# bigscience-workshop/petals

Hardware: AMD Instinct MI355X
Metric: single-batch generate tokens/sec, Llama-2-70B across 1/2/4/8 MI355X servers (higher is better)
Workload: dtype nf4-weights/bf16-compute; 1 GPU; model=llama-2-70b, global_batch=1, seq_len=363, prompt_len=128, parallelism=swarm-single, quant=nf4, stack=serve

## Files before the change

petals_amd/ops/csrc/bindings.cpp:

```cpp
#include <torch/extension.h>
#include <ATen/cuda/CUDAContext.h>

torch::Tensor rms_norm(torch::Tensor x, torch::Tensor w, double eps);
torch::Tensor rms_norm_f32out(torch::Tensor x, torch::Tensor w, double eps);
torch::Tensor layer_norm(torch::Tensor x, torch::Tensor w, torch::Tensor b, double eps);
torch::Tensor layer_norm_f32out(torch::Tensor x, torch::Tensor w, torch::Tensor b, double eps);
torch::Tensor swiglu(torch::Tensor gate, torch::Tensor up);
void warm_spin(int64_t microseconds);
std::vector<torch::Tensor> apply_rope(
    torch::Tensor q, torch::Tensor k, torch::Tensor cos_t, torch::Tensor sin_t, torch::Tensor pos);
void rope_cache_write(
    torch::Tensor qkv, torch::Tensor cos_t, torch::Tensor sin_t, torch::Tensor pos,
    torch::Tensor k_cache, torch::Tensor v_cache, int64_t qh, int64_t kh);
void kv_cache_write(
    torch::Tensor qkv, torch::Tensor pos,
    torch::Tensor k_cache, torch::Tensor v_cache, int64_t qh, int64_t kh);
void kv_cache_store_fp8(torch::Tensor new_kv, torch::Tensor cache, int64_t prefix_length);
torch::Tensor qkv_rope_reduce(
    torch::Tensor partials, c10::optional<torch::Tensor> cos_t, c10::optional<torch::Tensor> sin_t,
    torch::Tensor pos, torch::Tensor k_cache, torch::Tensor v_cache,
    int64_t qh, int64_t kh, bool rope, c10::optional<torch::Tensor> bias);
torch::Tensor gemv_bf16(
    torch::Tensor wt, torch::Tensor x, torch::Tensor workspace,
    c10::optional<torch::Tensor> residual, int64_t epilogue, int64_t splits_override,
    c10::optional<torch::Tensor> bias);
torch::Tensor attn_decode_fused(
    torch::Tensor q, torch::Tensor k_cache, torch::Tensor v_cache, torch::Tensor kv_len,
    int64_t gq, int64_t n_splits, torch::Tensor part_o, torch::Tensor part_ml, double scale,
    c10::optional<torch::Tensor> alibi_slopes);
torch::Tensor attn_prefill_fused(
    torch::Tensor q, torch::Tensor k, torch::Tensor v,
    int64_t kv_len, int64_t kv_offset, double scale, bool causal,
    c10::optional<torch::Tensor> alibi_slopes);
std::vector<torch::Tensor> nf4_quantize(torch::Tensor w);
torch::Tensor gemv_int8(
    torch::Tensor q, torch::Tensor scale, torch::Tensor x, torch::Tensor workspace,
    c10::optional<torch::Tensor> residual, int64_t epilogue, int64_t splits_override,
    c10::optional<torch::Tensor> bias);
torch::Tensor nf4_dequantize(torch::Tensor packed, torch::Tensor absmax);
torch::Tensor gemv_nf4(
    torch::Tensor packed, torch::Tensor absmax, torch::Tensor x, torch::Tensor workspace,
    c10::optional<torch::Tensor> residual, int64_t epilogue, int64_t splits_override,
    c10::optional<torch::Tensor> bias, c10::optional<torch::Tensor> absmax_t);
torch::Tensor gemv_bf16_moe(
    torch::Tensor wt_all, torch::Tensor x, torch::Tensor sel, int64_t k_per_tok,
    torch::Tensor workspace, int64_t epilogue, int64_t splits_override);
torch::Tensor gemv_nf4_moe(
    torch::Tensor packed_all, torch::Tensor absmax_all, torch::Tensor x, torch::Tensor sel,
    int64_t k_per_tok, torch::Tensor workspace, int64_t epilogue, int64_t splits_override);
torch::Tensor moe_gemm(
    c10::optional<torch::Tensor> wt_all, c10::optional<torch::Tensor> packed_all,
    c10::optional<torch::Tensor> absmax_all, torch::Tensor x, torch::Tensor sorted_pairs,
    torch::Tensor tile_expert, int64_t k_per_tok, int64_t n_rows,
    c10::optional<torch::Tensor> q8_all, c10::optional<torch::Tensor> scale8_all);
torch::Tensor gemv_int8_moe(
    torch::Tensor q8_all, torch::Tensor scale8_all, torch::Tensor x, torch::Tensor sel,
    int64_t k_per_tok, torch::Tensor workspace, int64_t epilogue, int64_t splits_override);
int64_t gemv_int8_moe_splits(int64_t in_dim, int64_t out_dim, int64_t rows, int64_t splits_override);
torch::Tensor gemm_nf4(
    torch::Tensor packed, torch::Tensor absmax, torch::Tensor x, c10::optional<torch::Tensor> bias);
torch::Tensor gemm_int8(
    torch::Tensor q8, torch::Tensor scale8, torch::Tensor x, c10::optional<torch::Tensor> bias);
std::vector<torch::Tensor> mxfp4_quantize(torch::Tensor w);
torch::Tensor mxfp4_dequantize(torch::Tensor packed, torch::Tensor scales);
torch::Tensor gemv_mxfp4(
    torch::Tensor packed, torch::Tensor scales, torch::Tensor x, torch::Tensor workspace,
    c10::optional<torch::Tensor> residual, int64_t epilogue, int64_t splits_override,
    c10::optional<torch::Tensor> bias);
int64_t gemv_mxfp4_splits(int64_t in_dim, int64_t out_dim, int64_t batch, int64_t splits_override);
torch::Tensor gemm_mxfp4(
    torch::Tensor packed, torch::Tensor scales, torch::Tensor x, c10::optional<torch::Tensor> bias);

PYBIND11_MODULE(TORCH_EXTENSION_NAME, m) {
  m.def("rms_norm", &rms_norm, "RMSNorm (bf16 -> bf16)");
  m.def("rms_norm_f32out", &rms_norm_f32out, "RMSNorm (bf16 -> f32)");
  m.def("layer_norm", &layer_norm, "LayerNorm with weight+bias (bf16 -> bf16)");
  m.def("layer_norm_f32out", &layer_norm_f32out, "LayerNorm with weight+bias (bf16 -> f32)");
  m.def("swiglu", &swiglu, "silu(gate) * up (bf16)");
  m.def("warm_spin", &warm_spin, "occupy the device queue for ~N us (keep-warm)");
  m.def("apply_rope", &apply_rope, "rotate q,k by positions (bf16)");
  m.def("rope_cache_write", &rope_cache_write, "fused decode rope + kv cache write");
  m.def("kv_cache_write", &kv_cache_write, "decode kv cache write without rope (ALiBi families)");
  m.def("kv_cache_store_fp8", &kv_cache_store_fp8,
        "prefill write bf16 [B, KV, S, hd] -> float8_e4m3fn cache rows [prefix, prefix+S) "
        "(saturating, round to nearest even)",
        py::arg("new_kv"), py::arg("cache"), py::arg("prefix_length"));
  m.def("qkv_rope_reduce", &qkv_rope_reduce,
        "fused qkv split-K reduce + rope + kv-cache write (consumes RAW gemv partials)",
        py::arg("partials"), py::arg("cos_t"), py::arg("sin_t"), py::arg("pos"),
        py::arg("k_cache"), py::arg("v_cache"), py::arg("qh"), py::arg("kh"), py::arg("rope") = true,
        py::arg("bias") = py::none());
  m.def("gemv_bf16", &gemv_bf16, "split-K bf16 gemv with fused epilogue",
        py::arg("wt"), py::arg("x"), py::arg("workspace"), py::arg("residual"), py::arg("epilogue"),
        py::arg("splits") = 0, py::arg("bias") = py::none());
  m.def("attn_decode_fused", &attn_decode_fused, "GQA decode attention (flash-decoding)",
        py::arg("q"), py::arg("k_cache"), py::arg("v_cache"), py::arg("kv_len"), py::arg("gq"),
        py::arg("n_splits"), py::arg("part_o"), py::arg("part_ml"), py::arg("scale"),
        py::arg("alibi_slopes") = py::none());
  m.def("attn_prefill_fused", &attn_prefill_fused, "MFMA flash prefill attention (bf16, causal, GQA)",
        py::arg("q"), py::arg("k"), py::arg("v"), py::arg("kv_len"), py::arg("kv_offset"),
        py::arg("scale"), py::arg("causal"), py::arg("alibi_slopes") = py::none());
  m.def("gemv_int8", &gemv_int8, "split-K weight-only int8 gemv (per-column scales) with epilogue",
        py::arg("q"), py::arg("scale"), py::arg("x"), py::arg("workspace"),
        py::arg("residual"), py::arg("epilogue"), py::arg("splits") = 0, py::arg("bias") = py::none());
  m.def("nf4_quantize", &nf4_quantize, "blockwise NF4 quantize [in,out] bf16 -> (packed u8, absmax bf16)");
  m.def("nf4_dequantize", &nf4_dequantize, "NF4 -> bf16");
  m.def("gemv_nf4", &gemv_nf4, "split-K NF4 gemv (dequant fused) with epilogue",
        py::arg("packed"), py::arg("absmax"), py::arg("x"), py::arg("workspace"),
        py::arg("residual"), py::arg("epilogue"), py::arg("splits") = 0, py::arg("bias") = py::none(),
        py::arg("absmax_t") = py::none());
  m.def("gemv_bf16_moe", &gemv_bf16_moe,
        "device-routed MoE gemv: stacked bf16 expert weights, expert ids from a device tensor",
        py::arg("wt_all"), py::arg("x"), py::arg("sel"), py::arg("k_per_tok"),
        py::arg("workspace"), py::arg("epilogue"), py::arg("splits") = 0);
  m.def("gemv_nf4_moe", &gemv_nf4_moe,
        "device-routed MoE gemv: stacked NF4 expert weights, expert ids from a device tensor",
        py::arg("packed_all"), py::arg("absmax_all"), py::arg("x"), py::arg("sel"),
        py::arg("k_per_tok"), py::arg("workspace"), py::arg("epilogue"), py::arg("splits") = 0);
  m.def("moe_gemm", &moe_gemm,
        "grouped MFMA GEMM over expert-sorted (token, slot) pairs (prefill; NF4/int8 dequant "
        "fused into the LDS B-tile staging); exactly one of wt_all / packed_all / q8_all",
        py::arg("wt_all"), py::arg("packed_all"), py::arg("absmax_all"), py::arg("x"),
        py::arg("sorted_pairs"), py::arg("tile_expert"), py::arg("k_per_tok"), py::arg("n_rows"),
        py::arg("q8_all") = py::none(), py::arg("scale8_all") = py::none());
  m.def("gemv_int8_moe", &gemv_int8_moe,
        "device-routed MoE gemv: stacked int8 expert weights (per-column scales), expert ids "
        "from a device tensor",
        py::arg("q8_all"), py::arg("scale8_all"), py::arg("x"), py::arg("sel"),
        py::arg("k_per_tok"), py::arg("workspace"), py::arg("epilogue"), py::arg("splits") = 0);
  m.def("gemv_int8_moe_splits", &gemv_int8_moe_splits,
        "split count gemv_int8_moe uses for (in, out, rows) — sizes the workspace",
        py::arg("in_dim"), py::arg("out_dim"), py::arg("rows"), py::arg("splits") = 0);
  m.def("gemm_nf4", &gemm_nf4,
        "dense prefill MFMA GEMM x[M,in] @ NF4 W[in,out] (+bias) -> bf16, dequant fused into the "
        "LDS staging",
        py::arg("packed"), py::arg("absmax"), py::arg("x"), py::arg("bias") = py::none());
  m.def("gemm_int8", &gemm_int8,
        "dense prefill MFMA GEMM x[M,in] @ int8 W[in,out] (+bias) -> bf16, column scale in the "
        "epilogue",
        py::arg("q8"), py::arg("scale8"), py::arg("x"), py::arg("bias") = py::none());
  m.def("mxfp4_quantize", &mxfp4_quantize,
        "OCP MXFP4 quantize [in,out] bf16 -> (packed u8 [in/2,out], E8M0 scales u8 [in/32,out])");
  m.def("mxfp4_dequantize", &mxfp4_dequantize, "MXFP4 -> bf16 [in,out]");
  m.def("gemv_mxfp4", &gemv_mxfp4,
        "split-K MXFP4 gemv (hardware fp4 dequant, E8M0 block scales) with epilogue",
        py::arg("packed"), py::arg("scales"), py::arg("x"), py::arg("workspace"),
        py::arg("residual"), py::arg("epilogue"), py::arg("splits") = 0, py::arg("bias") = py::none());
  m.def("gemv_mxfp4_splits", &gemv_mxfp4_splits,
        "split count gemv_mxfp4 uses for (in, out, batch) — sizes the workspace",
        py::arg("in_dim"), py::arg("out_dim"), py::arg("batch"), py::arg("splits") = 0);
  m.def("gemm_mxfp4", &gemm_mxfp4,
        "dense prefill MFMA GEMM x[M,in] @ MXFP4 W[in,out] (+bias) -> bf16, hardware fp4 dequant "
        "fused into the LDS staging",
        py::arg("packed"), py::arg("scales"), py::arg("x"), py::arg("bias") = py::none());
}
```

petals_amd/ops/csrc/nf4.hip:

```cpp

#include "common.h"
#include "gemv_reduce.h"
#include <torch/extension.h>
#include <ATen/cuda/CUDAContext.h>

__device__ __constant__ float NF4_LUT_C[16] = {
    -1.0f, -0.6961928009986877f, -0.5250730514526367f, -0.39491748809814453f,
    -0.28444138169288635f, -0.18477343022823334f, -0.09105003625154495f, 0.0f,
    0.07958029955625534f, 0.16093020141124725f, 0.24611230194568634f,
    0.33791524171829224f, 0.4407098293304443f, 0.5626170039176941f,
    0.7229568362236023f, 1.0f};


__global__ void nf4_quantize_kernel(
    const unsigned short* __restrict__ w,
    unsigned char* __restrict__ packed,
    unsigned short* __restrict__ absmax,
    long n_blocks,
    int out_dim) {
  const long blk = (long)blockIdx.x * blockDim.x + threadIdx.x;
  if (blk >= n_blocks) return;
  const long base = blk * 64;
  float vals[64];
  float amax = 0.f;
#pragma unroll
  for (int j = 0; j < 64; ++j) {
    vals[j] = bf16_to_f32(w[base + j]);
    amax = fmaxf(amax, fabsf(vals[j]));
  }
  const float amax_bf = bf16_to_f32(f32_to_bf16(amax));
  absmax[blk] = f32_to_bf16(amax);
  const float inv = amax_bf > 0.f ? 1.0f / amax_bf : 0.f;
#pragma unroll
  for (int j = 0; j < 32; ++j) {
    unsigned char lo, hi;
#pragma unroll
    for (int half = 0; half < 2; ++half) {
      const float v = vals[2 * j + half] * inv;
      int best = 0;
      float bd = fabsf(v - NF4_LUT_C[0]);
#pragma unroll
      for (int l = 1; l < 16; ++l) {
        const float d = fabsf(v - NF4_LUT_C[l]);
        if (d < bd) { bd = d; best = l; }
      }
      if (half == 0) lo = (unsigned char)best; else hi = (unsigned char)best;
    }
    packed[blk * 32 + j] = (unsigned char)(lo | (hi << 4));
  }
}


__global__ void nf4_dequant_kernel(
    const unsigned char* __restrict__ packed,
    const unsigned short* __restrict__ absmax,
    unsigned short* __restrict__ out,
    long n_elems) {
  const long i = ((long)blockIdx.x * blockDim.x + threadIdx.x) * 2;
  if (i >= n_elems) return;
  const unsigned char byte = packed[i >> 1];
  const float scale = bf16_to_f32(absmax[i >> 6]);
  out[i] = f32_to_bf16(NF4_LUT_C[byte & 0xF] * scale);
  if (i + 1 < n_elems) out[i + 1] = f32_to_bf16(NF4_LUT_C[byte >> 4] * scale);
}


#define NF4_OPL 8
#define NF4_OUT_PER_WAVE (WAVE * NF4_OPL)

template <int BATCH>
__global__ __launch_bounds__(WAVE) void gemv_nf4_kernel(
    const unsigned char* __restrict__ packed,
    const unsigned short* __restrict__ absmax,
    const unsigned short* __restrict__ absmax_t,
    const float* __restrict__ x,
    float* __restrict__ partials,
    int in_dim,
    int out_dim,
    int i_per_split) {
  __shared__ float2 lut2[256];
  for (int i = threadIdx.x; i < 256; i += blockDim.x)
    lut2[i] = make_float2(NF4_LUT_C[i & 0xF], NF4_LUT_C[i >> 4]);
  __syncthreads();

  constexpr int OPL = NF4_OPL;
  const int lane = threadIdx.x & (WAVE - 1);
  const int out0 = blockIdx.x * (WAVE * OPL) + lane * OPL;
  if (out0 >= out_dim) return;
  const int split = blockIdx.y;
  const int i_begin = split * i_per_split;
  const int i_end = min(i_begin + i_per_split, in_dim);
  const bool full = (out0 + OPL) <= out_dim;

  float acc[BATCH][OPL];
#pragma unroll
  for (int b = 0; b < BATCH; ++b)
#pragma unroll
    for (int v = 0; v < OPL; ++v) acc[b][v] = 0.f;

  if (full) {
    constexpr int UNROLL = (BATCH > 4) ? 8 : 16;
    const int half_out = out_dim >> 1;
    const unsigned char* pp = packed + (size_t)i_begin * half_out + (out0 >> 1);
    const unsigned short* amt = absmax_t ? absmax_t + (size_t)(out0 >> 6) * in_dim : nullptr;
    int i = i_begin;
    for (; i + UNROLL <= i_end; i += UNROLL) {
      unsigned int pk[UNROLL];
#pragma unroll
      for (int u = 0; u < UNROLL; ++u)
        pk[u] = *reinterpret_cast<const unsigned int*>(pp + (size_t)u * half_out);
      float am[UNROLL];
      if (amt) {
#pragma unroll
        for (int c8 = 0; c8 < UNROLL / 8; ++c8) {
          const short8 a8 = *reinterpret_cast<const short8*>(amt + i + c8 * 8);
#pragma unroll
          for (int e = 0; e < 8; ++e) am[c8 * 8 + e] = bf16_to_f32((unsigned short)a8[e]);
        }
      } else {
#pragma unroll
        for (int u = 0; u < UNROLL; ++u)
          am[u] = bf16_to_f32(absmax[(size_t)(i + u) * (out_dim >> 6) + (out0 >> 6)]);
      }
      float xs[BATCH][UNROLL];
#pragma unroll
      for (int b = 0; b < BATCH; ++b)
#pragma unroll
        for (int u = 0; u < UNROLL; ++u)
          xs[b][u] = x[(size_t)b * in_dim + i + u];
#pragma unroll
      for (int u = 0; u < UNROLL; ++u) {
        float wf[OPL];
#pragma unroll
        for (int p2 = 0; p2 < 4; ++p2) {
          const float2 w2 = lut2[(pk[u] >> (8 * p2)) & 0xFFu];
          wf[2 * p2] = w2.x;
          wf[2 * p2 + 1] = w2.y;
        }
#pragma unroll
        for (int b = 0; b < BATCH; ++b) {
          const float xa = xs[b][u] * am[u];
#pragma unroll
          for (int v = 0; v < OPL; ++v) acc[b][v] = fmaf(wf[v], xa, acc[b][v]);
        }
      }
      pp += (size_t)UNROLL * half_out;
    }
    for (; i < i_end; ++i) {
      const float am = bf16_to_f32(absmax[(size_t)i * (out_dim >> 6) + (out0 >> 6)]);
#pragma unroll
      for (int b = 0; b < BATCH; ++b) {
        const float xa = x[(size_t)b * in_dim + i] * am;
        const unsigned int wd =
            *reinterpret_cast<const unsigned int*>(packed + (size_t)i * half_out + (out0 >> 1));
#pragma unroll
        for (int p2 = 0; p2 < 4; ++p2) {
          const float2 w2 = lut2[(wd >> (8 * p2)) & 0xFFu];
          acc[b][2 * p2] = fmaf(w2.x, xa, acc[b][2 * p2]);
          acc[b][2 * p2 + 1] = fmaf(w2.y, xa, acc[b][2 * p2 + 1]);
        }
      }
    }
  } else {
    for (int i = i_begin; i < i_end; ++i) {
      const float am = bf16_to_f32(absmax[(size_t)i * (out_dim >> 6) + (out0 >> 6)]);
#pragma unroll
      for (int b = 0; b < BATCH; ++b) {
        const float xa = x[(size_t)b * in_dim + i] * am;
#pragma unroll
        for (int v = 0; v < OPL; ++v) {
          if (out0 + v < out_dim) {
            const unsigned char byte = packed[(size_t)i * (out_dim >> 1) + ((out0 + v) >> 1)];
            const float2 w2 = lut2[byte];
            acc[b][v] = fmaf(((out0 + v) & 1) ? w2.y : w2.x, xa, acc[b][v]);
          }
        }
      }
    }
  }

#pragma unroll
  for (int b = 0; b < BATCH; ++b) {
    float* dst = partials + ((size_t)split * BATCH + b) * out_dim + out0;
    if (full) {
#pragma unroll
      for (int q = 0; q < OPL / 4; ++q)
        reinterpret_cast<float4v*>(dst)[q] =
            float4v{acc[b][4 * q], acc[b][4 * q + 1], acc[b][4 * q + 2], acc[b][4 * q + 3]};
    } else {
#pragma unroll
      for (int v = 0; v < OPL; ++v)
        if (out0 + v < out_dim) dst[v] = acc[b][v];
    }
  }
}


std::vector<torch::Tensor> nf4_quantize(torch::Tensor w) {
  TORCH_CHECK(w.is_cuda() && w.dtype() == torch::kBFloat16 && w.dim() == 2);
  TORCH_CHECK(w.size(1) % 64 == 0, "out dim must be a multiple of 64");
  auto wc = w.contiguous();
  const long in_dim = wc.size(0), out_dim = wc.size(1);
  const long n_blocks = in_dim * out_dim / 64;
  auto packed = torch::empty({in_dim, out_dim / 2}, w.options().dtype(torch::kUInt8));
  auto absmax = torch::empty({in_dim, out_dim / 64}, w.options());
  auto stream = at::cuda::getCurrentCUDAStream();
  const long blocks = (n_blocks + 255) / 256;
  nf4_quantize_kernel<<<blocks, 256, 0, stream>>>(
      reinterpret_cast<const unsigned short*>(wc.data_ptr()),
      packed.data_ptr<unsigned char>(),
      reinterpret_cast<unsigned short*>(absmax.data_ptr()),
      n_blocks, (int)out_dim);
  HIP_CHECK_LAST();
  return {packed, absmax};
}

torch::Tensor nf4_dequantize(torch::Tensor packed, torch::Tensor absmax) {
  TORCH_CHECK(packed.is_cuda() && packed.dtype() == torch::kUInt8 && packed.dim() == 2);
  const long in_dim = packed.size(0), half_out = packed.size(1);
  const long n = in_dim * half_out * 2;
  auto out = torch::empty({in_dim, half_out * 2}, absmax.options());
  auto stream = at::cuda::getCurrentCUDAStream();
  const long blocks = (n / 2 + 255) / 256;
  nf4_dequant_kernel<<<blocks, 256, 0, stream>>>(
      packed.data_ptr<unsigned char>(),
      reinterpret_cast<const unsigned short*>(absmax.data_ptr()),
      reinterpret_cast<unsigned short*>(out.data_ptr()), n);
  HIP_CHECK_LAST();
  return out;
}

torch::Tensor gemv_nf4(
    torch::Tensor packed,
    torch::Tensor absmax,
    torch::Tensor x,
    torch::Tensor workspace,
    c10::optional<torch::Tensor> residual,
    int64_t epilogue,
    int64_t splits_override,
    c10::optional<torch::Tensor> bias,
    c10::optional<torch::Tensor> absmax_t) {
  TORCH_CHECK(packed.is_cuda() && packed.dtype() == torch::kUInt8);
  TORCH_CHECK(x.dtype() == torch::kFloat32 && x.dim() == 2);
  const int in_dim = packed.size(0);
  const int out_dim = packed.size(1) * 2;
  const int batch = x.size(0);
  TORCH_CHECK(x.size(1) == in_dim && batch <= 8, "NF4 decode gemv supports batch <= 8");

  const long out_waves = (out_dim + (long)NF4_OUT_PER_WAVE - 1) / NF4_OUT_PER_WAVE;
  long splits = splits_override > 0 ? splits_override : (1536 + out_waves - 1) / out_waves;
  long max_splits = (in_dim + 31) / 32;
  if (splits > max_splits) splits = max_splits;
  if (splits < 1) splits = 1;
  const int i_per_split = (int)(((in_dim + splits - 1) / splits + 15L) & ~15L);
  splits = (in_dim + i_per_split - 1) / i_per_split;

  torch::Tensor partials;
  auto f32opts = x.options().dtype(torch::kFloat32);
  if (workspace.numel() >= (int64_t)splits * batch * out_dim) {
    partials = workspace;
  } else {
    partials = torch::empty({(int64_t)splits, batch, out_dim}, f32opts);
  }
  dim3 grid(out_waves, splits);
  auto stream = at::cuda::getCurrentCUDAStream();

  const unsigned short* amt_p = nullptr;
  if (absmax_t.has_value() && absmax_t->defined() && absmax_t->numel() > 0) {
    TORCH_CHECK(absmax_t->is_contiguous() && absmax_t->size(0) == out_dim / 64
                && absmax_t->size(1) == in_dim);
    amt_p = reinterpret_cast<const unsigned short*>(absmax_t->data_ptr());
  }
#define LAUNCH_NF4(B)                                                         \
  case B:                                                                     \
    gemv_nf4_kernel<B><<<grid, WAVE, 0, stream>>>(                            \
        packed.data_ptr<unsigned char>(),                                     \
        reinterpret_cast<const unsigned short*>(absmax.data_ptr()), amt_p,    \
        x.data_ptr<float>(), partials.data_ptr<float>(), in_dim, out_dim, i_per_split); \
    break;
  switch (batch) {
    LAUNCH_NF4(1) LAUNCH_NF4(2) LAUNCH_NF4(3) LAUNCH_NF4(4)
    LAUNCH_NF4(5) LAUNCH_NF4(6) LAUNCH_NF4(7) LAUNCH_NF4(8)
  }
#undef LAUNCH_NF4
  HIP_CHECK_LAST();

  if (epilogue < 0) {
    return partials.view(-1).narrow(0, 0, (int64_t)splits * batch * out_dim)
        .view({(int64_t)splits, (int64_t)batch, (int64_t)out_dim});
  }
  return launch_gemv_reduce(
      partials, residual, bias, (int)splits, batch, out_dim, (int)epilogue, f32opts,
      absmax.options());
}
```

petals_amd/ops/fused_decode.py:

```python

from __future__ import annotations

import math
import os
from typing import Dict, Optional, Tuple

import torch

from petals_amd.ops import reference

_EPI_RAW = -1
_EPI_PLAIN_F32 = 0
_EPI_PLAIN_BF16 = 1
_EPI_RESIDUAL_BF16 = 2
_EPI_SWIGLU_F32 = 3
_EPI_GELU_F32 = 4

_workspaces: Dict[Tuple[torch.device, str], torch.Tensor] = {}
_retired_workspaces: list = []


def _get_ws(device: torch.device, key: str, numel: int) -> torch.Tensor:
    k = (device, key)
    ws = _workspaces.get(k)
    if ws is None or ws.numel() < numel:
        if ws is not None:
            _retired_workspaces.append(ws)
        ws = torch.empty(numel, dtype=torch.float32, device=device)
        _workspaces[k] = ws
    return ws


class DecodeContext:

    def __init__(self, device: torch.device):
        self.pos = torch.zeros(1, dtype=torch.int32, device=device)
        self.kv_len = torch.zeros(1, dtype=torch.int32, device=device)

    def set_position(self, prefix_length: int) -> None:
        self.pos.fill_(prefix_length)
        self.kv_len.fill_(prefix_length + 1)

    def advance(self) -> None:
        self.pos.add_(1)
        self.kv_len.add_(1)


_split_autotune_cache: Dict[Tuple[str, int, int], int] = {}

_PREFILL_GEMM_MODES = ("dense", "fused")


def prefill_gemm_mode() -> str:
    mode = os.environ.get("PETALS_AMD_PREFILL_GEMM", "dense")
    if mode not in _PREFILL_GEMM_MODES:
        raise ValueError(
            f"PETALS_AMD_PREFILL_GEMM={mode!r}: expected one of {', '.join(_PREFILL_GEMM_MODES)}"
        )
    return mode


def set_prefill_gemm_mode(mode: str) -> None:
    if mode not in _PREFILL_GEMM_MODES:
        raise ValueError(f"prefill_gemm={mode!r}: expected one of {', '.join(_PREFILL_GEMM_MODES)}")
    os.environ["PETALS_AMD_PREFILL_GEMM"] = mode


FUSED_GEMM_MAX_ROWS = {"nf4": 256, "int8": 512, "mxfp4": 256}


def fused_gemm_eligible(quant: str, rows: int, in_dim: int, out_dim: int) -> bool:
    return (
        quant in FUSED_GEMM_MAX_ROWS
        and 1 <= rows <= FUSED_GEMM_MAX_ROWS[quant]
        and in_dim % 64 == 0
        and out_dim % 64 == 0
    )


class _FastWeight:

    def __init__(self, t_bf16: torch.Tensor, hip, quant: str):
        self.hip = hip
        self.quant = quant
        self.in_dim, self.out_dim = t_bf16.shape
        self.t = self.packed = self.absmax = self.absmax_t = self.q8 = self.scale8 = None
        self.mx_packed = self.mx_scales = None
        if quant == "mxfp4":
            from petals_amd.ops import mxfp4

            mxfp4.check_shape(self.in_dim, self.out_dim)
            if t_bf16.is_cuda:
                self.mx_packed, self.mx_scales = hip.mxfp4_quantize(t_bf16.to(torch.bfloat16).contiguous())
            else:
                self.mx_packed, self.mx_scales = mxfp4.quantize(t_bf16.to(torch.bfloat16))
        elif quant == "nf4":
            self.packed, self.absmax = hip.nf4_quantize(t_bf16.contiguous())
            self.absmax_t = self.absmax.t().contiguous()
        elif quant == "int8":
            w = t_bf16.float()
            scale = w.abs().amax(dim=0).clamp_min(1e-8) / 127.0
            self.q8 = torch.round(w / scale).clamp(-127, 127).to(torch.int8).contiguous()
            self.scale8 = scale.to(torch.bfloat16).contiguous()
        else:
            self.t = t_bf16.contiguous()
        self.splits = self._autotune(t_bf16.device)

    def _autotune(self, device) -> int:
        key = (self.quant, self.in_dim, self.out_dim)
        if key in _split_autotune_cache:
            return _split_autotune_cache[key]
        if device.type != "cuda":
            return 0
        import time

        if self.quant == "nf4":
            candidates = [0, 32, 64, 96, 128, 160, 192, 256, 320, 384]
            max_chunk = 32
        elif self.quant == "int8":
            candidates = [0, 16, 32, 64, 128, 192]
            max_chunk = 128
        elif self.quant == "mxfp4":
            candidates = [0, 8, 16, 24, 32, 48, 64]
            max_chunk = 32
        else:
            candidates = [0, 8, 16, 32, 64, 128]
            max_chunk = 64
        candidates = [s for s in candidates if s == 0 or s * max_chunk <= self.in_dim]
        x = torch.randn(1, self.in_dim, device=device)
        ws = _get_ws(device, "gemv", 64 * max(self.out_dim, 1))
        best, best_t = 0, float("inf")
        for s in candidates:
            try:
                self._gemv_raw(x, ws, None, 0, s)
                torch.cuda.synchronize()
                t0 = time.perf_counter()
                for _ in range(8):
                    self._gemv_raw(x, ws, None, 0, s)
                torch.cuda.synchronize()
                dt = time.perf_counter() - t0
            except RuntimeError:
                continue
            if dt < best_t:
                best, best_t = s, dt
        _split_autotune_cache[key] = best
        return best

    @property
    def shape(self):
        return (self.in_dim, self.out_dim)

    def _gemv_raw(self, x, ws, residual, epilogue, splits, bias=None):
        if self.quant == "nf4":
            return self.hip.gemv_nf4(self.packed, self.absmax, x, ws, residual, epilogue, splits, bias,
                                     self.absmax_t)
        if self.quant == "int8":
            return self.hip.gemv_int8(self.q8, self.scale8, x, ws, residual, epilogue, splits, bias)
        if self.quant == "mxfp4":
            return self.hip.gemv_mxfp4(self.mx_packed, self.mx_scales, x, ws, residual, epilogue, splits, bias)
        return self.hip.gemv_bf16(self.t, x, ws, residual, epilogue, splits, bias)

    def gemv(self, x, ws, residual, epilogue, bias=None):
        return self._gemv_raw(x, ws, residual, epilogue, self.splits, bias)

    def dense(self) -> torch.Tensor:
        if self.quant == "nf4":
            return _dequant_cached(self, lambda: self.hip.nf4_dequantize(self.packed, self.absmax))
        if self.quant == "int8":
            return _dequant_cached(
                self, lambda: (self.q8.to(torch.float32) * self.scale8.float()).to(torch.bfloat16)
            )
        if self.quant == "mxfp4":
            if not self.mx_packed.is_cuda:
                from petals_amd.ops import mxfp4

                return mxfp4.dequantize(self.mx_packed, self.mx_scales)
            return _dequant_cached(self, lambda: self.hip.mxfp4_dequantize(self.mx_packed, self.mx_scales))
        return self.t

    def matmul(self, x: torch.Tensor, bias: Optional[torch.Tensor] = None) -> torch.Tensor:
        if (
            prefill_gemm_mode() == "fused"
            and not (torch.is_grad_enabled() and x.requires_grad)
            and x.is_cuda
            and x.dtype == torch.bfloat16
            and fused_gemm_eligible(self.quant, x.numel() // max(x.shape[-1], 1), self.in_dim, self.out_dim)
        ):
            x2 = x.reshape(-1, self.in_dim).contiguous()
            if self.quant == "nf4":
                out = self.hip.gemm_nf4(self.packed, self.absmax, x2, bias)
            elif self.quant == "mxfp4":
                out = self.hip.gemm_mxfp4(self.mx_packed, self.mx_scales, x2, bias)
            else:
                out = self.hip.gemm_int8(self.q8, self.scale8, x2, bias)
            return out.view(*x.shape[:-1], self.out_dim)
        out = torch.matmul(x, self.dense())
        return out if bias is None else out + bias


_dequant_cache: "OrderedDict[int, torch.Tensor]" = None
_dequant_cache_bytes = 0


def _dequant_cache_budget() -> int:
    import os as _os

    return int(_os.environ.get("PETALS_AMD_DEQUANT_CACHE_MB", "16384")) << 20


def _dequant_cached(w, make) -> torch.Tensor:
    global _dequant_cache, _dequant_cache_bytes
    from collections import OrderedDict

    if _dequant_cache is None:
        _dequant_cache = OrderedDict()
    key = id(w)
    t = _dequant_cache.get(key)
    if t is not None:
        _dequant_cache.move_to_end(key)
        return t
    t = make()
    budget = _dequant_cache_budget()
    nbytes = t.numel() * t.element_size()
    if nbytes > budget:
        return t
    while _dequant_cache and _dequant_cache_bytes + nbytes > budget:
        _k, old = _dequant_cache.popitem(last=False)
        _dequant_cache_bytes -= old.numel() * old.element_size()
    _dequant_cache[key] = t
    _dequant_cache_bytes += nbytes
    import weakref

    def _evict(k=key):
        global _dequant_cache_bytes
        old = _dequant_cache.pop(k, None) if _dequant_cache else None
        if old is not None:
            _dequant_cache_bytes -= old.numel() * old.element_size()

    weakref.finalize(w, _evict)
    return t


def decode_step_auto(fast, hidden, k_cache, v_cache, prefix_length: int = -1, ctx=None, adapter=None,
                     max_b: int = 8):
    B = hidden.shape[0]
    if B <= max_b:
        return fast.decode_step(hidden, k_cache, v_cache, prefix_length, ctx=ctx, adapter=adapter)
    outs = []
    for i in range(0, B, max_b):
        outs.append(
            fast.decode_step(
                hidden[i : i + max_b], k_cache[i : i + max_b], v_cache[i : i + max_b],
                prefix_length, ctx=ctx, adapter=adapter,
            )
        )
    return torch.cat(outs, dim=0)


class _TPFastPathMixin:

    tp_world = 1
    tp_group = None

    @staticmethod
    def _mm_autograd(w: "_FastWeight", x: torch.Tensor, bias: Optional[torch.Tensor] = None) -> torch.Tensor:
        out = torch.matmul(x, w.dense())
        return out if bias is None else out + bias

    def _tp_copy(self, x: torch.Tensor) -> torch.Tensor:
        if self.tp_world <= 1:
            return x
        from petals_amd.parallel.tp import copy_to_tp

        return copy_to_tp(x, self.tp_group)

    def _tp_allreduce_(self, t: torch.Tensor) -> None:
        import torch.distributed as dist

        dist.all_reduce(t, op=dist.ReduceOp.SUM, group=self.tp_group)

    def _tp_reduce(self, x: torch.Tensor) -> torch.Tensor:
        if self.tp_world <= 1:
            return x
        from petals_amd.parallel.tp import reduce_from_tp

        return reduce_from_tp(x, self.tp_group)


class LlamaFastPath(_TPFastPathMixin):
    graph_safe = True

    def __init__(self, block, hip_ops, quant: str = "none", tp_world: int = 1, tp_group=None):
        cfg = block.config
        self.hip = hip_ops
        self.cfg = cfg
        self.quant = quant
        self.tp_world = tp_world
        self.tp_group = tp_group
        if tp_world > 1:
            self.graph_safe = False
        self.hd = cfg.head_dim
        self.qh = cfg.num_attention_heads
        self.kh = cfg.n_kv_heads
        self.gq = self.qh // self.kh
        self.scale = 1.0 / math.sqrt(self.hd)
        self.eps = cfg.layer_norm_eps

        attn = block.self_attn
        device = attn.q_proj.weight.device

        def t(w):
            return w.detach().to(torch.bfloat16).t().contiguous()

        self.ln1_w = block.input_layernorm.weight.detach().to(torch.bfloat16).contiguous()
        self.ln2_w = block.post_attention_layernorm.weight.detach().to(torch.bfloat16).contiguous()
        self.wqkv_t = _FastWeight(
            torch.cat([t(attn.q_proj.weight), t(attn.k_proj.weight), t(attn.v_proj.weight)], dim=1),
            hip_ops, quant,
        )
        self.wo_t = _FastWeight(t(attn.o_proj.weight), hip_ops, quant)
        self._empty_bf16 = torch.empty(0, device=device, dtype=torch.bfloat16)
        for lin in (attn.q_proj, attn.k_proj, attn.v_proj, attn.o_proj):
            lin.weight.data = self._empty_bf16
        self.has_bias = attn.q_proj.bias is not None
        self._init_mlp_weights(block, hip_ops, quant)

        self.rope_cos: Optional[torch.Tensor] = None
        self.rope_sin: Optional[torch.Tensor] = None
        self._pos = torch.zeros(1, dtype=torch.int32, device=device)
        self._kv_len = torch.zeros(1, dtype=torch.int32, device=device)
        self.device = device
        self._empty_f32 = torch.empty(0, dtype=torch.float32, device=device)

    def _init_mlp_weights(self, block, hip_ops, quant):
        def t(w):
            return w.detach().to(torch.bfloat16).t().contiguous()

        mlp = block.mlp
        self.wgateup_t = _FastWeight(
            torch.cat([t(mlp.gate_proj.weight), t(mlp.up_proj.weight)], dim=1), hip_ops, quant
        )
        self.wdown_t = _FastWeight(t(mlp.down_proj.weight), hip_ops, quant)
        for lin in (mlp.gate_proj, mlp.up_proj, mlp.down_proj):
            lin.weight.data = self._empty_bf16

    def _mlp_dense(self, xn2, adapter, autograd: bool):
        xn2 = self._tp_copy(xn2)
        if autograd:
            gateup = torch.matmul(xn2, self.wgateup_t.dense())
        else:
            gateup = self.wgateup_t.matmul(xn2)
        inter = self.wgateup_t.shape[1] // 2
        gate, up = gateup[..., :inter], gateup[..., inter:]
        if adapter is not None:
            dg, du = adapter.delta("gate", xn2), adapter.delta("up", xn2)
            if dg is not None:
                gate = gate + dg
            if du is not None:
                up = up + du
        if autograd:
            act = reference.swiglu(gate, up).to(xn2.dtype)
            down = torch.matmul(act, self.wdown_t.dense())
        else:
            act = self.hip.swiglu(gate.contiguous(), up.contiguous())
            down = self.wdown_t.matmul(act)
        if adapter is not None:
            dd = adapter.delta("down", act)
            if dd is not None:
                down = down + dd
        return down

    def _ensure_rope(self, needed: int):
        if self.rope_cos is None or self.rope_cos.shape[0] < needed:
            cos, sin = reference.build_rope_cache(
                self.hd,
                max(needed, self.cfg.max_position_embeddings),
                theta=self.cfg.rope_theta,
                rope_scaling=self.cfg.rope_scaling,
            )
            self.rope_cos = cos.to(self.device, torch.float32).contiguous()
            self.rope_sin = sin.to(self.device, torch.float32).contiguous()


    @torch.inference_mode()
    def decode_step(
        self,
        hidden: torch.Tensor,
        k_cache: torch.Tensor,
        v_cache: torch.Tensor,
        prefix_length: int = -1,
        ctx: Optional[DecodeContext] = None,
        adapter=None,
    ) -> torch.Tensor:
        B = hidden.shape[0]
        H = hidden.shape[-1]
        h = hidden.view(B, H)
        if h.dtype != torch.bfloat16:
            h = h.to(torch.bfloat16)
        h = h.contiguous()
        if ctx is None:
            assert prefix_length >= 0
            self._ensure_rope(prefix_length + 1)
            self._pos.fill_(prefix_length)
            self._kv_len.fill_(prefix_length + 1)
            pos, kv_len = self._pos, self._kv_len
        else:
            self._ensure_rope(k_cache.shape[2])
            pos, kv_len = ctx.pos, ctx.kv_len
        ws = _get_ws(self.device, "gemv", 64 * B * self._max_gemv_out())

        if adapter is None:
            xn = self.hip.rms_norm_f32out(h, self.ln1_w, self.eps)
            parts = self.wqkv_t.gemv(xn, ws, None, _EPI_RAW)
            q = self.hip.qkv_rope_reduce(
                parts, self.rope_cos, self.rope_sin, pos, k_cache[:B], v_cache[:B],
                self.qh, self.kh, True,
            )
        else:
            xn = self.hip.rms_norm_f32out(h, self.ln1_w, self.eps)
            qkv = self.wqkv_t.gemv(xn, ws, None, _EPI_PLAIN_F32)
            self._apply_qkv_adapter(qkv, xn, adapter)
            self.hip.rope_cache_write(
                qkv, self.rope_cos, self.rope_sin, pos, k_cache[:B], v_cache[:B], self.qh, self.kh
            )
            q = qkv[:, : self.qh * self.hd].contiguous()
        attn = self.hip.attn_decode_fused(
            q, k_cache[:B], v_cache[:B], kv_len, self.gq, 0,
            self._empty_f32, self._empty_f32, self.scale,
        )
        if self.tp_world > 1:
            part = self.wo_t.gemv(attn, ws, None, _EPI_PLAIN_F32)
            self._tp_allreduce_(part)
            h2 = (h.float() + part).to(torch.bfloat16)
        elif adapter is not None:
            d = adapter.delta("o", attn)
            h2 = self.wo_t.gemv(attn, ws, h, _EPI_RESIDUAL_BF16)
            if d is not None:
                h2 = h2 + d.to(h2.dtype)
        else:
            h2 = self.wo_t.gemv(attn, ws, h, _EPI_RESIDUAL_BF16)
        xn2 = self.hip.rms_norm_f32out(h2, self.ln2_w, self.eps)
        h3 = self._mlp_decode(xn2, h2, ws, adapter)
        return h3.view(B, 1, H)

    def _max_gemv_out(self) -> int:
        return max(self.wgateup_t.shape[1], self.wqkv_t.shape[1], self.wo_t.shape[1])

    def _mlp_decode(self, xn2, h2, ws, adapter):
        if self.tp_world > 1:
            assert adapter is None, "LoRA on TP shards is served via the generic path"
            act = self.wgateup_t.gemv(xn2, ws, None, _EPI_SWIGLU_F32)
            part = self.wdown_t.gemv(act, ws, None, _EPI_PLAIN_F32)
            self._tp_allreduce_(part)
            return (h2.float() + part).to(torch.bfloat16)
        if adapter is None:
            act = self.wgateup_t.gemv(xn2, ws, None, _EPI_SWIGLU_F32)
            return self.wdown_t.gemv(act, ws, h2, _EPI_RESIDUAL_BF16)
        gateup = self.wgateup_t.gemv(xn2, ws, None, _EPI_PLAIN_F32)
        inter = self.wgateup_t.shape[1] // 2
        dg, du = adapter.delta("gate", xn2), adapter.delta("up", xn2)
        gate, up = gateup[:, :inter], gateup[:, inter:]
        if dg is not None:
            gate = gate + dg.float()
        if du is not None:
            up = up + du.float()
# ... 539 lines not shown
```

Before: 77.22 tokens/s.

## Add multi-wave workgroup NF4 gemv with in-LDS split reduction and cold-cache autotune

Adds an NF4 decode gemv kernel in which each workgroup holds several waves, each handling a different K chunk. The waves combine their partial sums in shared memory, so fewer split partials reach the global reduce and each block reuses its LUT setup. Nontemporal weight loads are optional. The autotuner picks between the old kernel and the 4/8/16-wave variants, with or without NT, by timing each cold-cache call after an L2 flush. The cost is a larger autotune search, more kernel instantiations, and a combine ordering that must stay consistent with the grouped reduce.

```diff
diff --git a/petals_amd/ops/csrc/bindings.cpp b/petals_amd/ops/csrc/bindings.cpp
--- a/petals_amd/ops/csrc/bindings.cpp
+++ b/petals_amd/ops/csrc/bindings.cpp
@@ -41,7 +41,8 @@
 torch::Tensor gemv_nf4(
     torch::Tensor packed, torch::Tensor absmax, torch::Tensor x, torch::Tensor workspace,
     c10::optional<torch::Tensor> residual, int64_t epilogue, int64_t splits_override,
-    c10::optional<torch::Tensor> bias, c10::optional<torch::Tensor> absmax_t);
+    c10::optional<torch::Tensor> bias, c10::optional<torch::Tensor> absmax_t,
+    int64_t wg_waves, bool nt);
 torch::Tensor gemv_bf16_moe(
     torch::Tensor wt_all, torch::Tensor x, torch::Tensor sel, int64_t k_per_tok,
     torch::Tensor workspace, int64_t epilogue, int64_t splits_override);
@@ -108,7 +109,7 @@
   m.def("gemv_nf4", &gemv_nf4, "split-K NF4 gemv (dequant fused) with epilogue",
         py::arg("packed"), py::arg("absmax"), py::arg("x"), py::arg("workspace"),
         py::arg("residual"), py::arg("epilogue"), py::arg("splits") = 0, py::arg("bias") = py::none(),
-        py::arg("absmax_t") = py::none());
+        py::arg("absmax_t") = py::none(), py::arg("wg_waves") = 0, py::arg("nt") = false);
   m.def("gemv_bf16_moe", &gemv_bf16_moe,
         "device-routed MoE gemv: stacked bf16 expert weights, expert ids from a device tensor",
         py::arg("wt_all"), py::arg("x"), py::arg("sel"), py::arg("k_per_tok"),
diff --git a/petals_amd/ops/csrc/nf4.hip b/petals_amd/ops/csrc/nf4.hip
--- a/petals_amd/ops/csrc/nf4.hip
+++ b/petals_amd/ops/csrc/nf4.hip
@@ -192,6 +192,155 @@
       for (int v = 0; v < OPL; ++v)
         if (out0 + v < out_dim) dst[v] = acc[b][v];
     }
+  }
+}
+
+
+#define NF4_RED_GROUPS 16
+static_assert(NF4_RED_GROUPS == GEMV_REDUCE_GROUPS, "the wg kernel mirrors the reduce's grouping");
+template <int BATCH, int WAVES, bool NT>
+__global__ __launch_bounds__(WAVE * WAVES) void gemv_nf4_wg_kernel(
+    const unsigned char* __restrict__ packed,
+    const unsigned short* __restrict__ absmax,
+    const unsigned short* __restrict__ absmax_t,
+    const float* __restrict__ x,
+    float* __restrict__ partials,
+    int in_dim,
+    int out_dim,
+    int i_per_split,
+    int n_splits) {
+  constexpr int OPL = NF4_OPL;
+  constexpr int UNROLL = 16;
+  constexpr int THREADS = WAVE * WAVES;
+  __shared__ float2 lut2[256];
+  __shared__ float comb[WAVES][BATCH][NF4_OUT_PER_WAVE];
+  for (int i = threadIdx.x; i < 256; i += THREADS)
+    lut2[i] = make_float2(NF4_LUT_C[i & 0xF], NF4_LUT_C[i >> 4]);
+  __syncthreads();
+
+  const int lane = threadIdx.x & (WAVE - 1);
+  const int wave = __builtin_amdgcn_readfirstlane(threadIdx.x >> 6);
+  const int out0 = blockIdx.x * (WAVE * OPL) + lane * OPL;
+  const int split = blockIdx.y;
+  const int chunk = split + NF4_RED_GROUPS * wave;
+  const int i_begin = chunk < n_splits ? chunk * i_per_split : in_dim;
+  const int i_end = min(i_begin + i_per_split, in_dim);
+  const bool live = out0 < out_dim;
+  const bool full = (out0 + OPL) <= out_dim;
+
+  float acc[BATCH][OPL];
+#pragma unroll
+  for (int b = 0; b < BATCH; ++b)
+#pragma unroll
+    for (int v = 0; v < OPL; ++v) acc[b][v] = 0.f;
+
+  if (full) {
+    const int half_out = out_dim >> 1;
+    const unsigned char* pp = packed + (size_t)i_begin * half_out + (out0 >> 1);
+    const unsigned short* amt = absmax_t ? absmax_t + (size_t)(out0 >> 6) * in_dim : nullptr;
+    int i = i_begin;
+    for (; i + UNROLL <= i_end; i += UNROLL) {
+      unsigned int pk[UNROLL];
+#pragma unroll
+      for (int u = 0; u < UNROLL; ++u) {
+        const unsigned int* wp = reinterpret_cast<const unsigned int*>(pp + (size_t)u * half_out);
+        pk[u] = NT ? __builtin_nontemporal_load(wp) : *wp;
+      }
+      float am[UNROLL];
+      if (amt) {
+#pragma unroll
+        for (int c8 = 0; c8 < UNROLL / 8; ++c8) {
+          const short8 a8 = *reinterpret_cast<const short8*>(amt + i + c8 * 8);
+#pragma unroll
+          for (int e = 0; e < 8; ++e) am[c8 * 8 + e] = bf16_to_f32((unsigned short)a8[e]);
+        }
+      } else {
+#pragma unroll
+        for (int u = 0; u < UNROLL; ++u)
+          am[u] = bf16_to_f32(absmax[(size_t)(i + u) * (out_dim >> 6) + (out0 >> 6)]);
+      }
+      float xs[BATCH][UNROLL];
+#pragma unroll
+      for (int b = 0; b < BATCH; ++b)
+#pragma unroll
+        for (int u = 0; u < UNROLL; ++u)
+          xs[b][u] = x[(size_t)b * in_dim + i + u];
+#pragma unroll
+      for (int u = 0; u < UNROLL; ++u) {
+        float wf[OPL];
+#pragma unroll
+        for (int p2 = 0; p2 < 4; ++p2) {
+          const float2 w2 = lut2[(pk[u] >> (8 * p2)) & 0xFFu];
+          wf[2 * p2] = w2.x;
+          wf[2 * p2 + 1] = w2.y;
+        }
+#pragma unroll
+        for (int b = 0; b < BATCH; ++b) {
+          const float xa = xs[b][u] * am[u];
+#pragma unroll
+          for (int v = 0; v < OPL; ++v) acc[b][v] = fmaf(wf[v], xa, acc[b][v]);
+        }
+      }
+      pp += (size_t)UNROLL * half_out;
+    }
+    for (; i < i_end; ++i) {
+      const float am = bf16_to_f32(absmax[(size_t)i * (out_dim >> 6) + (out0 >> 6)]);
+#pragma unroll
+      for (int b = 0; b < BATCH; ++b) {
+        const float xa = x[(size_t)b * in_dim + i] * am;
+        const unsigned int wd =
+            *reinterpret_cast<const unsigned int*>(packed + (size_t)i * half_out + (out0 >> 1));
+#pragma unroll
+        for (int p2 = 0; p2 < 4; ++p2) {
+          const float2 w2 = lut2[(wd >> (8 * p2)) & 0xFFu];
+          acc[b][2 * p2] = fmaf(w2.x, xa, acc[b][2 * p2]);
+          acc[b][2 * p2 + 1] = fmaf(w2.y, xa, acc[b][2 * p2 + 1]);
+        }
+      }
+    }
+  } else if (live) {
+    for (int i = i_begin; i < i_end; ++i) {
+      const float am = bf16_to_f32(absmax[(size_t)i * (out_dim >> 6) + (out0 >> 6)]);
+#pragma unroll
+      for (int b = 0; b < BATCH; ++b) {
+        const float xa = x[(size_t)b * in_dim + i] * am;
+#pragma unroll
+        for (int v = 0; v < OPL; ++v) {
+          if (out0 + v < out_dim) {
+            const unsigned char byte = packed[(size_t)i * (out_dim >> 1) + ((out0 + v) >> 1)];
+            const float2 w2 = lut2[byte];
+            acc[b][v] = fmaf(((out0 + v) & 1) ? w2.y : w2.x, xa, acc[b][v]);
+          }
+        }
+      }
+    }
+  }
+
+#pragma unroll
+  for (int b = 0; b < BATCH; ++b)
+#pragma unroll
+    for (int q = 0; q < OPL / 4; ++q)
+      reinterpret_cast<float4v*>(&comb[wave][b][lane * OPL])[q] =
+          float4v{acc[b][4 * q], acc[b][4 * q + 1], acc[b][4 * q + 2], acc[b][4 * q + 3]};
+  __syncthreads();
+  const int col0 = blockIdx.x * NF4_OUT_PER_WAVE;
+  const int m = (n_splits - split + NF4_RED_GROUPS - 1) / NF4_RED_GROUPS;
+#pragma unroll
+  for (int e = threadIdx.x; e < BATCH * NF4_OUT_PER_WAVE; e += THREADS) {
+    const int b = e / NF4_OUT_PER_WAVE;
+    const int c = e % NF4_OUT_PER_WAVE;
+    float a0 = 0.f, a1 = 0.f;
+#pragma unroll
+    for (int w = 0; w + 1 < WAVES; w += 2) {
+      if (w + 1 < m) {
+        a0 = __fadd_rn(a0, comb[w][b][c]);
+        a1 = __fadd_rn(a1, comb[w + 1][b][c]);
+      }
+    }
+    float s = __fadd_rn(a0, a1);
+    if (m & 1) s = __fadd_rn(comb[m - 1][b][c], s);
+    if (col0 + c < out_dim)
+      partials[((size_t)split * BATCH + b) * out_dim + col0 + c] = s;
   }
 }
 
@@ -239,13 +388,18 @@
     int64_t epilogue,
     int64_t splits_override,
     c10::optional<torch::Tensor> bias,
-    c10::optional<torch::Tensor> absmax_t) {
+    c10::optional<torch::Tensor> absmax_t,
+    int64_t wg_waves,
+    bool nt) {
   TORCH_CHECK(packed.is_cuda() && packed.dtype() == torch::kUInt8);
   TORCH_CHECK(x.dtype() == torch::kFloat32 && x.dim() == 2);
   const int in_dim = packed.size(0);
   const int out_dim = packed.size(1) * 2;
   const int batch = x.size(0);
   TORCH_CHECK(x.size(1) == in_dim && batch <= 8, "NF4 decode gemv supports batch <= 8");
+  TORCH_CHECK(wg_waves == 0 || wg_waves == 1 || wg_waves == 4 || wg_waves == 8 || wg_waves == 16,
+              "wg_waves must be 0, 1, 4, 8 or 16");
+  TORCH_CHECK(!nt || wg_waves > 1, "nt selects a load policy of the wg kernel: give wg_waves 4, 8 or 16");
 
   const long out_waves = (out_dim + (long)NF4_OUT_PER_WAVE - 1) / NF4_OUT_PER_WAVE;
   long splits = splits_override > 0 ? splits_override : (1536 + out_waves - 1) / out_waves;
@@ -254,6 +408,10 @@
   if (splits < 1) splits = 1;
   const int i_per_split = (int)(((in_dim + splits - 1) / splits + 15L) & ~15L);
   splits = (in_dim + i_per_split - 1) / i_per_split;
+  const int waves = (wg_waves > 1 && batch <= 4 && splits <= NF4_RED_GROUPS * wg_waves
+                     && !(wg_waves == 16 && batch == 4)) ? (int)wg_waves : 1;
+  const int n_chunks = (int)splits;
+  if (waves > 1 && splits > NF4_RED_GROUPS) splits = NF4_RED_GROUPS;
 
   torch::Tensor partials;
   auto f32opts = x.options().dtype(torch::kFloat32);
@@ -278,10 +436,35 @@
         reinterpret_cast<const unsigned short*>(absmax.data_ptr()), amt_p,    \
         x.data_ptr<float>(), partials.data_ptr<float>(), in_dim, out_dim, i_per_split); \
     break;
-  switch (batch) {
-    LAUNCH_NF4(1) LAUNCH_NF4(2) LAUNCH_NF4(3) LAUNCH_NF4(4)
-    LAUNCH_NF4(5) LAUNCH_NF4(6) LAUNCH_NF4(7) LAUNCH_NF4(8)
-  }
+#define LAUNCH_NF4_WG(B, W, N)                                                \
+  gemv_nf4_wg_kernel<B, W, N><<<grid, WAVE * W, 0, stream>>>(                 \
+      packed.data_ptr<unsigned char>(),                                       \
+      reinterpret_cast<const unsigned short*>(absmax.data_ptr()), amt_p,      \
+      x.data_ptr<float>(), partials.data_ptr<float>(), in_dim, out_dim, i_per_split, n_chunks)
+#define LAUNCH_NF4_WG_W(B, W) \
+  do { if (nt) LAUNCH_NF4_WG(B, W, true); else LAUNCH_NF4_WG(B, W, false); } while (0)
+#define LAUNCH_NF4_WG_B(B)                                                    \
+  case B:                                                                     \
+    if (waves == 4) LAUNCH_NF4_WG_W(B, 4);                                    \
+    else if (waves == 8) LAUNCH_NF4_WG_W(B, 8);                               \
+    else LAUNCH_NF4_WG_W(B, 16);                                              \
+    break;
+  if (waves > 1) {
+    switch (batch) {
+      LAUNCH_NF4_WG_B(1) LAUNCH_NF4_WG_B(2) LAUNCH_NF4_WG_B(3)
+      case 4:
+        if (waves == 4) LAUNCH_NF4_WG_W(4, 4); else LAUNCH_NF4_WG_W(4, 8);
+        break;
+    }
+  } else {
+    switch (batch) {
+      LAUNCH_NF4(1) LAUNCH_NF4(2) LAUNCH_NF4(3) LAUNCH_NF4(4)
+      LAUNCH_NF4(5) LAUNCH_NF4(6) LAUNCH_NF4(7) LAUNCH_NF4(8)
+    }
+  }
+#undef LAUNCH_NF4_WG_W
+#undef LAUNCH_NF4_WG_B
+#undef LAUNCH_NF4_WG
 #undef LAUNCH_NF4
   HIP_CHECK_LAST();
 
diff --git a/petals_amd/ops/fused_decode.py b/petals_amd/ops/fused_decode.py
--- a/petals_amd/ops/fused_decode.py
+++ b/petals_amd/ops/fused_decode.py
@@ -46,7 +46,10 @@
         self.kv_len.add_(1)
 
 
-_split_autotune_cache: Dict[Tuple[str, int, int], int] = {}
+_split_autotune_cache: Dict[Tuple[str, int, int], object] = {}
+_COLD_FLUSH_BYTES = 512 << 20
+_COLD_ROUNDS = 15
+_NF4_WG_MAX_BATCH = 1
 
 _PREFILL_GEMM_MODES = ("dense", "fused")
 
@@ -79,6 +82,8 @@
 
 
 class _FastWeight:
+
+    wg_waves, nt = 0, False
 
     def __init__(self, t_bf16: torch.Tensor, hip, quant: str):
         self.hip = hip
@@ -104,9 +109,10 @@
             self.scale8 = scale.to(torch.bfloat16).contiguous()
         else:
             self.t = t_bf16.contiguous()
-        self.splits = self._autotune(t_bf16.device)
-
-    def _autotune(self, device) -> int:
+        tuned = self._autotune(t_bf16.device)
+        self.wg_waves, self.splits, self.nt = tuned if isinstance(tuned, tuple) else (0, tuned, False)
+
+    def _autotune(self, device):
         key = (self.quant, self.in_dim, self.out_dim)
         if key in _split_autotune_cache:
             return _split_autotune_cache[key]
@@ -143,8 +149,40 @@
                 continue
             if dt < best_t:
                 best, best_t = s, dt
+        if self.quant == "nf4":
+            best = self._autotune_nf4_policy(device, best)
         _split_autotune_cache[key] = best
         return best
+
+    def _autotune_nf4_policy(self, device, splits: int) -> Tuple[int, int, bool]:
+        candidates = [(0, splits, False)]
+        for waves in (4, 8, 16):
+            candidates += [(waves, splits, False), (waves, splits, True)]
+        x = torch.randn(1, self.in_dim, device=device)
+        ws = _get_ws(device, "gemv", 64 * max(self.out_dim, 1))
+        flush = torch.zeros(_COLD_FLUSH_BYTES // 4, dtype=torch.int32, device=device)
+
+        def run(cand):
+            waves, s, nt = cand
+            return self.hip.gemv_nf4(self.packed, self.absmax, x, ws, None, 0, s, None, self.absmax_t, waves, nt)
+
+        def cold_call(cand):
+            flush.sum()
+            t0, t1 = torch.cuda.Event(enable_timing=True), torch.cuda.Event(enable_timing=True)
+            t0.record()
+            run(cand)
+            t1.record()
+            t1.synchronize()
+            return t0.elapsed_time(t1)
+
+        for cand in candidates:
+            run(cand)
+        times = {cand: [] for cand in candidates}
+        for _ in range(_COLD_ROUNDS):
+            for cand in candidates:
+                times[cand].append(cold_call(cand))
+        med = {cand: sorted(t)[len(t) // 2] for cand, t in times.items()}
+        return min(med, key=med.get)
 
     @property
     def shape(self):
@@ -161,6 +199,9 @@
         return self.hip.gemv_bf16(self.t, x, ws, residual, epilogue, splits, bias)
 
     def gemv(self, x, ws, residual, epilogue, bias=None):
+        if self.quant == "nf4" and self.wg_waves > 1 and x.shape[0] <= _NF4_WG_MAX_BATCH:
+            return self.hip.gemv_nf4(self.packed, self.absmax, x, ws, residual, epilogue, self.splits, bias,
+                                     self.absmax_t, self.wg_waves, self.nt)
         return self._gemv_raw(x, ws, residual, epilogue, self.splits, bias)
 
     def dense(self) -> torch.Tensor:
```

New measurement: 83.40 tokens/s (median of 6 runs). 8.0% higher.
